# XiaoHan-Git/RO-MAP

Hardware: AMD Instinct MI355X
Metric: ray-samples/sec (train: hash-encode->MLP->composite fwd+bwd+optimizer) per object-NeRF (higher is better)
Workload: dtype fp16 params/activations, fp32 accumulate + fp32 master; 1 GPU; OfflineNeRF-style training, 1 synthetic 'room'-like object per GPU, base.json defaults (hash L=16 F=2 T=2^16, MLP 64x1), R=4096 rays x S=32 samples/step, 40 views 640x480 resident in HBM; objects=1, samples_per_ray=32, backend=1, parallelism=object-per-GPU (no training collective; RCCL gather-to-root of the final render), launcher=single process, ranks_in_collective=1, visible_devices=1

## Files before the change

### ro-map_amd/csrc/kernels_encode.hip

```cpp
#include "device_common.h"
#include "model.h"
#include "batch_device.h"
#include "encode_device.h"
#include "tile_device.h"
#include "store_policy.h"
#include "xorwow.h"
#ifdef MON_OVERLAP_PROBE
#include <hip/hip_ext.h>
#endif

namespace mon {

constexpr uint32_t kEncLdsBytes = 163840;
static_assert(kEncWholeMax == kEncLdsBytes / 4u, "model.h: a whole-level tile is the CU's LDS");
constexpr uint32_t kEncParityMax = 65536u;
constexpr uint32_t kEncWgPerLevel = 16;
constexpr uint32_t kEncSpt = 8;
constexpr uint32_t kEncThreads = kTileThreads;

bool encode_tiles_supported(const LevelTable& lt, const NetDims& nd) {
    if (nd.L < 1 || nd.L > kMaxLevels) return false;
    for (int l = 0; l < nd.L; ++l) { const uint32_t size = lt.offset[l + 1] - lt.offset[l]; if (size > kEncParityMax || (size & 7u)) return false; }
    return (nd.n_mlp & 7u) == 0u;
}

__global__ void __launch_bounds__(256) k_sample_points(BatchPtrs b, ObjectConst oc, DevState* __restrict__ st, float4_t* __restrict__ x_all, LiveArgs live) {
    __shared__ PointsLds lds;
    const uint32_t R = oc.R, nwords = R >> 6, iter = st->iter;
    const uint32_t nvalid = points_prefix(lds, b.mask, nwords);
    if (blockIdx.x == 0u && threadIdx.x == 0u) st->n_valid_pre = nvalid;
    if (nvalid == 0u) return;
    const uint32_t s = blockIdx.x * blockDim.x + threadIdx.x;
    if (s >= R * 32u) return;
    if (live.occ_bits) points_sample<true>(lds, b, oc, iter, nvalid, nwords, s, x_all, live);
    else points_sample<false>(lds, b, oc, iter, nvalid, nwords, s, x_all);
}
__global__ void __launch_bounds__(64) k_live_reset(const DevState* __restrict__ st, uint32_t* __restrict__ cnt) {
    if (threadIdx.x < kLiveMaxParts) cnt[((size_t)(st->iter & 1u) * kLiveMaxParts + threadIdx.x) * kLiveCntStride] = 0u;
}

struct EncodeArgs {
    LevelFast lt; int L; uint32_t n_mlp;
    const uint16_t* half_tiles;
    const float4_t* x_all;
    half2_t* e_soa;
    uint32_t B, spw;
    const DevState* st;
    uint32_t gen_next; BatchPtrs b_next; DatasetPtrs ds;  ObjectConst oc;
    LiveArgs live;
};

__device__ __forceinline__ half2_t enc_chain(const uint32_t (&c0)[4], const uint32_t (&c1)[4], const float (&pos)[3]) {
    const float2_t wx = { 1.f - pos[0], pos[0] };
    const float wy[2] = { 1.f - pos[1], pos[1] }, wz[2] = { 1.f - pos[2], pos[2] };
    const float2_t wxy[2] = { wx * wy[0], wx * wy[1] };
    float2_t a = { 0.f, 0.f };
#pragma unroll
    for (int j = 0; j < 4; ++j) {
        const float2_t w = wxy[j & 1] * wz[j >> 1];
        const half2_t v0 = __builtin_bit_cast(half2_t, c0[j]), v1 = __builtin_bit_cast(half2_t, c1[j]);
        a = __builtin_elementwise_fma(float2_t{ w.x, w.x }, float2_t{ (float)v0.x, (float)v0.y }, a);
        a = __builtin_elementwise_fma(float2_t{ w.y, w.y }, float2_t{ (float)v1.x, (float)v1.y }, a);
    }
    return half2_t{ (half_t)a.x, (half_t)a.y };
}

template <bool LIVE>
__device__ __forceinline__ void load_positions(float4_t (&xs)[kEncSpt], uint32_t (&slot)[kEncSpt], const EncodeArgs& a, uint32_t s_base, uint32_t s_end,
        uint32_t count) {
    if constexpr (LIVE) {
#pragma unroll
        for (uint32_t k = 0; k < kEncSpt; ++k) { const uint32_t j = threadIdx.x + k * kEncThreads; slot[k] = (j < count) ? a.live.idx[s_base + j] : 0xffffffffu; }
#pragma unroll
        for (uint32_t k = 0; k < kEncSpt; ++k) xs[k] = a.x_all[slot[k] != 0xffffffffu ? slot[k] : s_base];
    } else {
#pragma unroll
        for (uint32_t k = 0; k < kEncSpt; ++k) { const uint32_t s = s_base + threadIdx.x + k * kEncThreads; slot[k] = s < s_end ? s : 0xffffffffu;
            xs[k] = a.x_all[min(s, s_end - 1u)]; }
    }
}
template <bool LIVE> __device__ __forceinline__ bool round_on(uint32_t k, uint32_t count) {
    return !LIVE || k * kEncThreads + (threadIdx.x & ~63u) < count; }

template <bool HASHED, bool POW2, bool LIVE>
__device__ __forceinline__ void encode_whole(const uint32_t* tile, const EncodeArgs& a, uint32_t s_base, uint32_t s_end, uint32_t count,
        half2_t* __restrict__ out, float scale, uint32_t size, uint32_t my, uint32_t mz, uint32_t mask) {
    if (s_base + threadIdx.x >= s_end && !LIVE) return;
    float4_t xs[kEncSpt]; uint32_t slot[kEncSpt]; load_positions<LIVE>(xs, slot, a, s_base, s_end, count);
#pragma unroll
    for (uint32_t k = 0; k < kEncSpt; ++k) {
        if (!round_on<LIVE>(k, count)) continue;
        uint32_t i0[4], i1[4], c0[4], c1[4]; float pos[3];
        enc_indices<HASHED, POW2>(xs[k], scale, size, my, mz, mask, i0, i1, pos);
#pragma unroll
        for (int j = 0; j < 4; ++j) { c0[j] = tile[i0[j]]; c1[j] = tile[i1[j]]; }
        const half2_t e = enc_chain(c0, c1, pos);
        if (slot[k] != 0xffffffffu) policy_store<MON_SP_E>(e, out + slot[k]);
    }
}

template <bool HASHED, bool POW2, bool LIVE>
__device__ __forceinline__ void encode_parity(uint32_t* tile, const uint4* __restrict__ src, const EncodeArgs& a, uint32_t s_base, uint32_t s_end, uint32_t count,
                                              half2_t* __restrict__ out, float scale, uint32_t size, uint32_t my, uint32_t mz, uint32_t mask) {
    uint32_t veven[kEncSpt][4], cache[kEncSpt][2]; float pos[kEncSpt][3];
    const bool walk = LIVE ? (threadIdx.x & ~63u) < count : s_base + threadIdx.x < s_end;
    float4_t xs[kEncSpt]; uint32_t slot[kEncSpt];
    if (walk) load_positions<LIVE>(xs, slot, a, s_base, s_end, count);
    __builtin_amdgcn_s_waitcnt(0x0f70);
    __syncthreads();
    if (walk) {
#pragma unroll
        for (uint32_t k = 0; k < kEncSpt; ++k) {
            if (!round_on<LIVE>(k, count)) continue;
            uint32_t i0[4], i1[4], c[4];
            enc_indices<HASHED, POW2>(xs[k], scale, size, my, mz, mask, i0, i1, pos[k]);
#pragma unroll
            for (int j = 0; j < 4; ++j) {
                const bool odd0 = (i0[j] & 1u) != 0u;
                const uint32_t ev = odd0 ? i1[j] : i0[j], od = odd0 ? i0[j] : i1[j];
                veven[k][j] = tile[ev >> 1];
                c[j] = (od & 0xfffeu) | (odd0 ? 1u : 0u);
            }
            cache[k][0] = c[0] | (c[1] << 16); cache[k][1] = c[2] | (c[3] << 16);
        }
    }
    __syncthreads();
    tile_copy(tile, src + size / 8u, size / 8u);
    __builtin_amdgcn_s_waitcnt(0x0f70);
    __syncthreads();
    if (walk) {
#pragma unroll
        for (uint32_t k = 0; k < kEncSpt; ++k) {
            if (!round_on<LIVE>(k, count)) continue;
            uint32_t c0[4], c1[4];
#pragma unroll
            for (int j = 0; j < 4; ++j) {
                const uint32_t c = (j & 1) ? (cache[k][j >> 1] >> 16) : (cache[k][j >> 1] & 0xffffu);
                const uint32_t vodd = tile[c >> 1];
                const bool odd0 = (c & 1u) != 0u;
                c0[j] = odd0 ? vodd : veven[k][j]; c1[j] = odd0 ? veven[k][j] : vodd;
            }
            const half2_t e = enc_chain(c0, c1, pos[k]);
            if (slot[k] != 0xffffffffu) policy_store<MON_SP_E>(e, out + slot[k]);
        }
    }
}

__global__ void __launch_bounds__(kEncThreads) k_encode_tiles(EncodeArgs a) {
    extern __shared__ __attribute__((aligned(16))) unsigned char smem[];
    uint32_t* tile = reinterpret_cast<uint32_t*>(smem);
    const uint32_t level = blockIdx.x / kEncWgPerLevel, part = blockIdx.x - level * kEncWgPerLevel;
    if (a.gen_next && level == 0u && blockIdx.y == 0u && threadIdx.x < 256u)
        for (uint32_t c0 = part * 256u; c0 < a.oc.R; c0 += kEncWgPerLevel * 256u) gen_candidate(a.b_next, a.ds, a.oc, a.st->n_boxes, a.st->iter + 1u,
                c0 + threadIdx.x);
    const uint32_t w = blockIdx.y * kEncWgPerLevel + part;
    const uint32_t s_base = w * a.spw, s_end = min(s_base + a.spw, a.B);
    if (s_base >= a.B) return;
    const uint32_t off = a.lt.offset[level], size = a.lt.size[level], my = a.lt.my[level], mz = a.lt.mz[level], mask = a.lt.mask[level];
    const bool hashed = a.lt.hashed[level] != 0u, pow2 = mask != 0xffffffffu;
    const float scale = a.lt.scale[level];
    const uint4* src = reinterpret_cast<const uint4*>(a.half_tiles + 2u * (size_t)off);
    half2_t* out = a.e_soa + (size_t)level * a.B;
    tile_copy(tile, src, size <= kEncWholeMax ? size / 4u : size / 8u);
    const bool live = a.live.idx != nullptr;
    uint32_t cnt0 = 0u, cnt1 = 0u;
    if (live) { cnt0 = a.live.cnt[(size_t)w * kLiveCntStride]; cnt1 = a.live.cnt[((size_t)kLiveMaxParts + w) * kLiveCntStride]; }
    const uint32_t iter = a.st->iter;
    if (live && blockIdx.x == 0u && blockIdx.y == 0u && threadIdx.x < kLiveMaxParts)
        a.live.cnt[((size_t)((iter + 1u) & 1u) * kLiveMaxParts + threadIdx.x) * kLiveCntStride] = 0u;
    if (a.st->n_valid_pre == 0u) return;
    const uint32_t count = min((iter & 1u) ? cnt1 : cnt0, s_end - s_base);
#define MON_ENC_CALL(FN, H, P2, ...) do { if (live) FN<H, P2, true>(__VA_ARGS__); else FN<H, P2, false>(__VA_ARGS__); } while (0)
    if (size <= kEncWholeMax) {
        __builtin_amdgcn_s_waitcnt(0x0f70);
        __syncthreads();
        if (hashed) { if (pow2) MON_ENC_CALL(encode_whole, true, true, tile, a, s_base, s_end, count, out, scale, size, my, mz, mask);
            else MON_ENC_CALL(encode_whole, true, false, tile, a, s_base, s_end, count, out, scale, size, my, mz, mask); }
        else MON_ENC_CALL(encode_whole, false, false, tile, a, s_base, s_end, count, out, scale, size, my, mz, mask);
    } else {
        if (hashed) { if (pow2) MON_ENC_CALL(encode_parity, true, true, tile, src, a, s_base, s_end, count, out, scale, size, my, mz, mask);
            else MON_ENC_CALL(encode_parity, true, false, tile, src, a, s_base, s_end, count, out, scale, size, my, mz, mask); }
        else MON_ENC_CALL(encode_parity, false, false, tile, src, a, s_base, s_end, count, out, scale, size, my, mz, mask);
    }
#undef MON_ENC_CALL
}

__global__ void __launch_bounds__(256) k_build_tiles_image(LevelFast lt, int L, const uint32_t* __restrict__ grid ,
                                                           uint32_t* __restrict__ image) {
    const uint32_t e = blockIdx.x * blockDim.x + threadIdx.x;
    if (e >= lt.offset[L]) return;
    int lvl = 0;
#pragma unroll
    for (int l = 1; l < kMaxLevels; ++l) lvl += (l < L && e >= lt.offset[l]) ? 1 : 0;
    image[tile_slot(lt.offset[lvl], lt.size[lvl], e - lt.offset[lvl])] = grid[e];
}
void launch_build_tiles_image(hipStream_t s, const LevelFast& lf, const NetDims& nd, const uint16_t* params, uint16_t* half_tiles) {
    const uint32_t n = lf.offset[nd.L];
    hipLaunchKernelGGL(k_build_tiles_image, dim3((n + 255u) / 256u), dim3(256), 0, s, lf, nd.L, reinterpret_cast<const uint32_t*>(params + nd.n_mlp),
            reinterpret_cast<uint32_t*>(half_tiles));
}

__global__ void __launch_bounds__(256) k_xorwow_fill(XorwowState* __restrict__ states, uint32_t lanes, int flavour, uint32_t start,
                                                     float* __restrict__ out0, uint32_t n0, float* __restrict__ out1, uint32_t n1, float* __restrict__ out2,
                                                             uint32_t n2) {
    const uint32_t k = blockIdx.x * blockDim.x + threadIdx.x;
    if (k >= lanes) return;
    XorwowState st = states[k];
    uint32_t s = start;
    for (uint32_t j = (k + lanes - s) % lanes; j < n0; j += lanes) out0[j] = xorwow_uniform(xorwow_next(st), flavour);
    s = (uint32_t)(((uint64_t)s + n0) % lanes);
    for (uint32_t j = (k + lanes - s) % lanes; j < n1; j += lanes) out1[j] = xorwow_uniform(xorwow_next(st), flavour);
    s = (uint32_t)(((uint64_t)s + n1) % lanes);
    for (uint32_t j = (k + lanes - s) % lanes; j < n2; j += lanes) out2[j] = xorwow_uniform(xorwow_next(st), flavour);
    states[k] = st;
}
void launch_xorwow_fill(hipStream_t s, void* lane_states, uint32_t lanes, int flavour, uint32_t start, float* out0, uint32_t n0, float* out1, uint32_t n1,
        float* out2, uint32_t n2) {
    hipLaunchKernelGGL(k_xorwow_fill, dim3((lanes + 255u) / 256u), dim3(256), 0, s, reinterpret_cast<XorwowState*>(lane_states), lanes, flavour, start, out0,
            n0, out1, n1, out2, n2);
}

uint32_t encode_tiles_spw(uint32_t B) {
    const uint32_t per_chunk = kEncWgPerLevel * kEncThreads * kEncSpt, chunks = (B + per_chunk - 1u) / per_chunk;
    return (B + kEncWgPerLevel * chunks - 1u) / (kEncWgPerLevel * chunks);
}
void encode_tiles_setup_device() {
    hipFuncSetAttribute(reinterpret_cast<const void*>(&k_encode_tiles), hipFuncAttributeMaxDynamicSharedMemorySize, kEncLdsBytes); }

void launch_sample_points(hipStream_t s, const BatchPtrs& b, const ObjectConst& oc, DevState* st, float* x_all, const LiveArgs& live) {
    const uint32_t B = oc.R * 32u;
    if (live.occ_bits) hipLaunchKernelGGL(k_live_reset, dim3(1), dim3(64), 0, s, st, live.cnt);
    hipLaunchKernelGGL(k_sample_points, dim3((B + 255u) / 256u), dim3(256), 0, s, b, oc, st, reinterpret_cast<float4_t*>(x_all), live);
}

void launch_encode_tiles(hipStream_t s, const LevelFast& lf, const NetDims& nd, const uint16_t* half_tiles, const float* x_all, uint16_t* e_soa, uint32_t B,
        const DevState* st,
                         const BatchPtrs* b_next, const DatasetPtrs& ds, const ObjectConst& oc, uint32_t lds_bytes, const LiveArgs& live) {
    const uint32_t per_chunk = kEncWgPerLevel * kEncThreads * kEncSpt, chunks = (B + per_chunk - 1u) / per_chunk;
    const uint32_t spw = encode_tiles_spw(B);
    EncodeArgs a{ lf, nd.L, nd.n_mlp, half_tiles, reinterpret_cast<const float4_t*>(x_all), reinterpret_cast<half2_t*>(e_soa), B, spw, st,
            b_next ? 1u : 0u, b_next ? *b_next : BatchPtrs{}, ds, oc, live };
#ifdef MON_OVERLAP_PROBE
    if (lds_bytes & 1u) { hipExtLaunchKernelGGL(k_encode_tiles, dim3((uint32_t)nd.L * kEncWgPerLevel, chunks), dim3(kEncThreads), (lds_bytes & ~1u) ? (lds_bytes & ~1u)
            : kEncLdsBytes, s, nullptr, nullptr, hipExtAnyOrderLaunch, a); return; }
#endif
    hipLaunchKernelGGL(k_encode_tiles, dim3((uint32_t)nd.L * kEncWgPerLevel, chunks), dim3(kEncThreads), lds_bytes ? lds_bytes : kEncLdsBytes, s, a);
}

}
```

Before: 2.137 billion ray-samples/s.

## Vectorize hash-encode stores via quad DPP transpose and use fma_mix interpolation

In the hash-grid encode kernel, each lane now keeps four rounds of outputs and exchanges them across each lane quad with DPP swaps, so every lane writes one 16-byte vector store instead of four scattered 4-byte stores. The trilinear interpolation chain uses v_fma_mix_f32 inline asm, which reads fp16 halves directly and drops the explicit half-to-float conversions. For hashed power-of-two levels it computes byte offsets straight away to save the index shifts. Samples-per-workgroup is rounded up to a multiple of four to keep stores aligned, which can make the split across workgroups slightly uneven.

```diff
diff --git a/ro-map_amd/csrc/kernels_encode.hip b/ro-map_amd/csrc/kernels_encode.hip
--- a/ro-map_amd/csrc/kernels_encode.hip
+++ b/ro-map_amd/csrc/kernels_encode.hip
@@ -7,6 +7,13 @@
 #include "xorwow.h"
 #ifdef MON_OVERLAP_PROBE
 #include <hip/hip_ext.h>
+#endif
+
+#ifndef MON_ENC_WIDE_STORE
+#define MON_ENC_WIDE_STORE 1
+#endif
+#ifndef MON_ENC_MIX
+#define MON_ENC_MIX 1
 #endif
 
 namespace mon {
@@ -50,6 +57,34 @@
     LiveArgs live;
 };
 
+#if MON_ENC_MIX
+template <int HI, bool FIRST> __device__ __forceinline__ float enc_mix(float w, uint32_t v, float a) {
+    float r;
+    if constexpr (FIRST) {
+        if constexpr (HI) asm("v_fma_mix_f32 %0, %1, %2, 0 op_sel:[0,1,0] op_sel_hi:[0,1,0]" : "=v"(r) : "v"(w), "v"(v));
+        else asm("v_fma_mix_f32 %0, %1, %2, 0 op_sel:[0,0,0] op_sel_hi:[0,1,0]" : "=v"(r) : "v"(w), "v"(v));
+    } else {
+        if constexpr (HI) asm("v_fma_mix_f32 %0, %1, %2, %3 op_sel:[0,1,0] op_sel_hi:[0,1,0]" : "=v"(r) : "v"(w), "v"(v), "v"(a));
+        else asm("v_fma_mix_f32 %0, %1, %2, %3 op_sel:[0,0,0] op_sel_hi:[0,1,0]" : "=v"(r) : "v"(w), "v"(v), "v"(a));
+    }
+    return r;
+}
+__device__ __forceinline__ half2_t enc_chain(const uint32_t (&c0)[4], const uint32_t (&c1)[4], const float (&pos)[3]) {
+    const float2_t wx = { 1.f - pos[0], pos[0] };
+    const float wy[2] = { 1.f - pos[1], pos[1] }, wz[2] = { 1.f - pos[2], pos[2] };
+    const float2_t wxy[2] = { wx * wy[0], wx * wy[1] };
+    const float2_t w0 = wxy[0] * wz[0];
+    float ax = enc_mix<0, true>(w0.x, c0[0], 0.f), ay = enc_mix<1, true>(w0.x, c0[0], 0.f);
+    ax = enc_mix<0, false>(w0.y, c1[0], ax); ay = enc_mix<1, false>(w0.y, c1[0], ay);
+#pragma unroll
+    for (int j = 1; j < 4; ++j) {
+        const float2_t w = wxy[j & 1] * wz[j >> 1];
+        ax = enc_mix<0, false>(w.x, c0[j], ax); ay = enc_mix<1, false>(w.x, c0[j], ay);
+        ax = enc_mix<0, false>(w.y, c1[j], ax); ay = enc_mix<1, false>(w.y, c1[j], ay);
+    }
+    return half2_t{ (half_t)ax, (half_t)ay };
+}
+#else
 __device__ __forceinline__ half2_t enc_chain(const uint32_t (&c0)[4], const uint32_t (&c1)[4], const float (&pos)[3]) {
     const float2_t wx = { 1.f - pos[0], pos[0] };
     const float wy[2] = { 1.f - pos[1], pos[1] }, wz[2] = { 1.f - pos[2], pos[2] };
@@ -64,6 +99,43 @@
     }
     return half2_t{ (half_t)a.x, (half_t)a.y };
 }
+#endif
+
+template <int SH>
+__device__ __forceinline__ void enc_offsets_pow2(const float4_t& xv, float scale, uint32_t my, uint32_t mz, uint32_t mask, uint32_t (&o0)[4], uint32_t (&o1)[4],
+        float (&pos)[3]) {
+    uint32_t pg[3];
+#pragma unroll
+    for (int d = 0; d < 3; ++d) { const float q = fmaf(scale, xv[d], 0.5f); pg[d] = (uint32_t)floor_to_int(q); pos[d] = __builtin_amdgcn_fractf(q); }
+    const uint32_t mys = (my << SH) & 0xffffffu, mzs = (mz << SH) & 0xffffffu, masks = mask << SH, xs = pg[0] << SH;
+    const uint32_t y0 = __umul24(pg[1], mys), z0 = __umul24(pg[2], mzs);
+    const uint32_t ay[2] = { y0, y0 + mys }, az[2] = { z0, z0 + mzs };
+    const uint32_t dxm = (xs ^ (xs + (1u << SH))) & masks;
+#pragma unroll
+    for (int j = 0; j < 4; ++j) { o0[j] = (xs ^ ay[j & 1] ^ az[j >> 1]) & masks; o1[j] = o0[j] ^ dxm; }
+}
+__device__ __forceinline__ uint32_t tile_at(const uint32_t* tile, uint32_t byte_off) {
+    return *reinterpret_cast<const uint32_t*>(reinterpret_cast<const unsigned char*>(tile) + byte_off); }
+
+__device__ __forceinline__ void quad_transpose(uint32_t (&v)[4]) {
+    const bool b0 = (threadIdx.x & 1u) != 0u, b1 = (threadIdx.x & 2u) != 0u;
+    const auto swap1 = [](uint32_t x) { return (uint32_t)__builtin_amdgcn_mov_dpp((int)x, 0xB1, 0xf, 0xf, true); };
+    const auto swap2 = [](uint32_t x) { return (uint32_t)__builtin_amdgcn_mov_dpp((int)x, 0x4E, 0xf, 0xf, true); };
+#pragma unroll
+    for (int p = 0; p < 4; p += 2) { const uint32_t a = v[p], b = v[p + 1], pa = swap1(a), pb = swap1(b); v[p] = b0 ? pb : a; v[p + 1] = b0 ? b : pa; }
+#pragma unroll
+    for (int r = 0; r < 2; ++r) { const uint32_t a = v[r], b = v[r + 2], pa = swap2(a), pb = swap2(b); v[r] = b1 ? pb : a; v[r + 2] = b1 ? b : pa; }
+}
+__device__ __forceinline__ void store_quad_rounds(uint32_t (&q)[4], half2_t* __restrict__ out, uint32_t s0, uint32_t k0, uint32_t s_end) {
+    typedef uint32_t u32x4 __attribute__((ext_vector_type(4)));
+    quad_transpose(q);
+    const uint32_t s = s0 + (threadIdx.x & ~3u) + (k0 + (threadIdx.x & 3u)) * kEncThreads;
+    if (s + 4u <= s_end && (s & 3u) == 0u) policy_store<MON_SP_E>(u32x4{ q[0], q[1], q[2], q[3] }, reinterpret_cast<u32x4*>(out + s));
+    else {
+#pragma unroll
+        for (uint32_t m = 0; m < 4u; ++m) if (s + m < s_end) policy_store<MON_SP_E>(__builtin_bit_cast(half2_t, q[m]), out + s + m);
+    }
+}
 
 template <bool LIVE>
 __device__ __forceinline__ void load_positions(float4_t (&xs)[kEncSpt], uint32_t (&slot)[kEncSpt], const EncodeArgs& a, uint32_t s_base, uint32_t s_end,
@@ -79,29 +151,43 @@
             xs[k] = a.x_all[min(s, s_end - 1u)]; }
     }
 }
-template <bool LIVE> __device__ __forceinline__ bool round_on(uint32_t k, uint32_t count) {
-    return !LIVE || k * kEncThreads + (threadIdx.x & ~63u) < count; }
+__device__ __forceinline__ bool round_on(uint32_t k, uint32_t limit) { return k * kEncThreads + (threadIdx.x & ~63u) < limit; }
 
 template <bool HASHED, bool POW2, bool LIVE>
 __device__ __forceinline__ void encode_whole(const uint32_t* tile, const EncodeArgs& a, uint32_t s_base, uint32_t s_end, uint32_t count,
         half2_t* __restrict__ out, float scale, uint32_t size, uint32_t my, uint32_t mz, uint32_t mask) {
     if (s_base + threadIdx.x >= s_end && !LIVE) return;
+    constexpr bool WIDE = MON_ENC_WIDE_STORE && !LIVE, BYTES = MON_ENC_MIX && HASHED && POW2;
+    const uint32_t limit = LIVE ? count : s_end - s_base;
     float4_t xs[kEncSpt]; uint32_t slot[kEncSpt]; load_positions<LIVE>(xs, slot, a, s_base, s_end, count);
+    uint32_t q[4];
 #pragma unroll
     for (uint32_t k = 0; k < kEncSpt; ++k) {
-        if (!round_on<LIVE>(k, count)) continue;
-        uint32_t i0[4], i1[4], c0[4], c1[4]; float pos[3];
-        enc_indices<HASHED, POW2>(xs[k], scale, size, my, mz, mask, i0, i1, pos);
-#pragma unroll
-        for (int j = 0; j < 4; ++j) { c0[j] = tile[i0[j]]; c1[j] = tile[i1[j]]; }
-        const half2_t e = enc_chain(c0, c1, pos);
-        if (slot[k] != 0xffffffffu) policy_store<MON_SP_E>(e, out + slot[k]);
+        if (WIDE && (k & 3u) == 0u) q[0] = q[1] = q[2] = q[3] = 0u;
+        if (round_on(k, limit)) {
+            uint32_t i0[4], i1[4], c0[4], c1[4]; float pos[3];
+            if constexpr (BYTES) {
+                enc_offsets_pow2<2>(xs[k], scale, my, mz, mask, i0, i1, pos);
+#pragma unroll
+                for (int j = 0; j < 4; ++j) { c0[j] = tile_at(tile, i0[j]); c1[j] = tile_at(tile, i1[j]); }
+            } else {
+                enc_indices<HASHED, POW2>(xs[k], scale, size, my, mz, mask, i0, i1, pos);
+#pragma unroll
+                for (int j = 0; j < 4; ++j) { c0[j] = tile[i0[j]]; c1[j] = tile[i1[j]]; }
+            }
+            const half2_t e = enc_chain(c0, c1, pos);
+            if constexpr (WIDE) q[k & 3u] = __builtin_bit_cast(uint32_t, e);
+            else if (slot[k] != 0xffffffffu) policy_store<MON_SP_E>(e, out + slot[k]);
+        }
+        if (WIDE && (k & 3u) == 3u && round_on(k - 3u, limit)) store_quad_rounds(q, out, s_base, k - 3u, s_end);
     }
 }
 
 template <bool HASHED, bool POW2, bool LIVE>
 __device__ __forceinline__ void encode_parity(uint32_t* tile, const uint4* __restrict__ src, const EncodeArgs& a, uint32_t s_base, uint32_t s_end, uint32_t count,
                                               half2_t* __restrict__ out, float scale, uint32_t size, uint32_t my, uint32_t mz, uint32_t mask) {
+    constexpr bool WIDE = MON_ENC_WIDE_STORE && !LIVE, BYTES = MON_ENC_MIX && HASHED && POW2;
+    const uint32_t limit = LIVE ? count : s_end - s_base;
     uint32_t veven[kEncSpt][4], cache[kEncSpt][2]; float pos[kEncSpt][3];
     const bool walk = LIVE ? (threadIdx.x & ~63u) < count : s_base + threadIdx.x < s_end;
     float4_t xs[kEncSpt]; uint32_t slot[kEncSpt];
@@ -111,15 +197,26 @@
     if (walk) {
 #pragma unroll
         for (uint32_t k = 0; k < kEncSpt; ++k) {
-            if (!round_on<LIVE>(k, count)) continue;
+            if (!round_on(k, limit)) continue;
             uint32_t i0[4], i1[4], c[4];
-            enc_indices<HASHED, POW2>(xs[k], scale, size, my, mz, mask, i0, i1, pos[k]);
-#pragma unroll
-            for (int j = 0; j < 4; ++j) {
-                const bool odd0 = (i0[j] & 1u) != 0u;
-                const uint32_t ev = odd0 ? i1[j] : i0[j], od = odd0 ? i0[j] : i1[j];
-                veven[k][j] = tile[ev >> 1];
-                c[j] = (od & 0xfffeu) | (odd0 ? 1u : 0u);
+            if constexpr (BYTES) {
+                enc_offsets_pow2<1>(xs[k], scale, my, mz, mask, i0, i1, pos[k]);
+#pragma unroll
+                for (int j = 0; j < 4; ++j) {
+                    const bool odd0 = (i0[j] & 2u) != 0u;
+                    const uint32_t ev = odd0 ? i1[j] : i0[j], od = odd0 ? i0[j] : i1[j];
+                    veven[k][j] = tile_at(tile, ev);
+                    c[j] = ((od >> 1) & 0xfffeu) | (odd0 ? 1u : 0u);
+                }
+            } else {
+                enc_indices<HASHED, POW2>(xs[k], scale, size, my, mz, mask, i0, i1, pos[k]);
+#pragma unroll
+                for (int j = 0; j < 4; ++j) {
+                    const bool odd0 = (i0[j] & 1u) != 0u;
+                    const uint32_t ev = odd0 ? i1[j] : i0[j], od = odd0 ? i0[j] : i1[j];
+                    veven[k][j] = tile[ev >> 1];
+                    c[j] = (od & 0xfffeu) | (odd0 ? 1u : 0u);
+                }
             }
             cache[k][0] = c[0] | (c[1] << 16); cache[k][1] = c[2] | (c[3] << 16);
         }
@@ -129,19 +226,24 @@
     __builtin_amdgcn_s_waitcnt(0x0f70);
     __syncthreads();
     if (walk) {
+        uint32_t q[4];
 #pragma unroll
         for (uint32_t k = 0; k < kEncSpt; ++k) {
-            if (!round_on<LIVE>(k, count)) continue;
-            uint32_t c0[4], c1[4];
-#pragma unroll
-            for (int j = 0; j < 4; ++j) {
-                const uint32_t c = (j & 1) ? (cache[k][j >> 1] >> 16) : (cache[k][j >> 1] & 0xffffu);
-                const uint32_t vodd = tile[c >> 1];
-                const bool odd0 = (c & 1u) != 0u;
-                c0[j] = odd0 ? vodd : veven[k][j]; c1[j] = odd0 ? veven[k][j] : vodd;
+            if (WIDE && (k & 3u) == 0u) q[0] = q[1] = q[2] = q[3] = 0u;
+            if (round_on(k, limit)) {
+                uint32_t c0[4], c1[4];
+#pragma unroll
+                for (int j = 0; j < 4; ++j) {
+                    const uint32_t c = (j & 1) ? (cache[k][j >> 1] >> 16) : (cache[k][j >> 1] & 0xffffu);
+                    const uint32_t vodd = tile[c >> 1];
+                    const bool odd0 = (c & 1u) != 0u;
+                    c0[j] = odd0 ? vodd : veven[k][j]; c1[j] = odd0 ? veven[k][j] : vodd;
+                }
+                const half2_t e = enc_chain(c0, c1, pos[k]);
+                if constexpr (WIDE) q[k & 3u] = __builtin_bit_cast(uint32_t, e);
+                else if (slot[k] != 0xffffffffu) policy_store<MON_SP_E>(e, out + slot[k]);
             }
-            const half2_t e = enc_chain(c0, c1, pos[k]);
-            if (slot[k] != 0xffffffffu) policy_store<MON_SP_E>(e, out + slot[k]);
+            if (WIDE && (k & 3u) == 3u && round_on(k - 3u, limit)) store_quad_rounds(q, out, s_base, k - 3u, s_end);
         }
     }
 }
@@ -222,7 +324,7 @@
 
 uint32_t encode_tiles_spw(uint32_t B) {
     const uint32_t per_chunk = kEncWgPerLevel * kEncThreads * kEncSpt, chunks = (B + per_chunk - 1u) / per_chunk;
-    return (B + kEncWgPerLevel * chunks - 1u) / (kEncWgPerLevel * chunks);
+    return ((B + kEncWgPerLevel * chunks - 1u) / (kEncWgPerLevel * chunks) + 3u) & ~3u;
 }
 void encode_tiles_setup_device() {
     hipFuncSetAttribute(reinterpret_cast<const void*>(&k_encode_tiles), hipFuncAttributeMaxDynamicSharedMemorySize, kEncLdsBytes); }
```

Result: no change. 2.156 billion ray-samples/s, median of 6 (+0.9%).
